# ilpoviertola/V-AURA

Measured on AMD Instinct MI355X. Metric: audio codec tokens/sec (whole node), 2.56 s clips, higher is better.
Workload: dtype f16x2-split(22b)/f32-acc

## Files before the change

include/vaura_hip.h:

```cpp
#ifndef VAURA_HIP_H
#define VAURA_HIP_H

#include <stddef.h>
#include <stdint.h>

#ifdef __cplusplus
extern "C" {
#endif

typedef void* vaura_stream_t;

typedef enum vaura_status {
  VAURA_OK = 0,
  VAURA_ERR_ARG = -1,
  VAURA_ERR_SHAPE = -2,
  VAURA_ERR_DTYPE = -3,
  VAURA_ERR_STATE = -4
} vaura_status;

typedef enum vaura_wdtype { VAURA_W_F32 = 0, VAURA_W_BF16 = 1, VAURA_W_FP8 = 2, VAURA_W_H1 = 3, VAURA_W_H2 = 4, VAURA_W_FP8H = 5 } vaura_wdtype;

typedef struct vaura_dims {
  int32_t n_layer;
  int32_t d_model;
// ... 213 lines not shown
  const vaura_vit_block* blocks_host;
  const float *norm_w, *norm_b;
  const float* agg_cls;
  const float *agg_ln1_w, *agg_ln1_b, *agg_ln2_w, *agg_ln2_b;
  const void* agg_in_w; const float* agg_in_b;
  const void* agg_out_w; const float* agg_out_b;
  const void* agg_l1_w; const float* agg_l1_b;
  const void* agg_l2_w; const float* agg_l2_b;
  float* ws_x; float* ws_qkv; uint16_t* ws_a; uint16_t* ws_h; uint16_t* ws_p; float* ws_z; float* ws_s;
} vaura_vit;
int vaura_avclip_forward(const vaura_vit* v, const float* frames, int n_seg, float* feats, vaura_stream_t s);
size_t vaura_avclip_workspace_bytes(const vaura_vit* v, int n_seg, int which);

void vaura_set_debug_flags(unsigned flags);
void vaura_set_debug_flags2(unsigned flags);
long long vaura_debug_counter(int which);

const char* vaura_version(void);
size_t vaura_struct_size(int which);

#ifdef __cplusplus
}
#endif
#endif
```

vaura_amd/_lib.py:

```python
from __future__ import annotations

import ctypes as C
import os
from typing import Optional

_HERE = os.path.dirname(os.path.abspath(__file__))
LIB_PATH = os.path.join(_HERE, "csrc", "libvaura_hip.so")

W_F32, W_BF16, W_FP8, W_H1, W_H2, W_FP8H = 0, 1, 2, 3, 4, 5
EPI_STORE, EPI_RESID, EPI_SWIGLU, EPI_GELU, EPI_LOGITS = 0, 1, 2, 3, 4
KERNEL_KINDS = ("embed", "qkv", "attn", "wo", "w13", "w2", "heads", "sample")

c_float_p = C.c_void_p


class Dims(C.Structure):
    _fields_ = [("n_layer", C.c_int32), ("d_model", C.c_int32), ("n_head", C.c_int32), ("ffn_dim", C.c_int32),
                ("n_codebooks", C.c_int32), ("vocab", C.c_int32), ("cond_dim", C.c_int32), ("tok_dim", C.c_int32),
                ("cond_in", C.c_int32), ("codebook_dim", C.c_int32), ("tokens_per_frame", C.c_int32),
                ("eps", C.c_float)]


class LayerWeights(C.Structure):
    _fields_ = [("wqkv", C.c_void_p), ("wo", C.c_void_p), ("w13", C.c_void_p), ("w2", C.c_void_p),
# ... 78 lines not shown

SIGNATURES = {
    "vaura_audio_normalize": (C.c_int, [C.c_void_p, C.c_void_p, C.c_int, C.c_int64, C.c_int, C.c_int, C.c_float, C.c_float,
                                        C.c_void_p, C.c_void_p]),
    "vaura_audio_scratch_elems": (C.c_size_t, [C.c_int]),
    "vaura_audio_loudness": (C.c_int, [C.c_void_p, C.c_void_p, C.c_int, C.c_int64, C.c_int, C.c_float, C.c_int, C.c_float, C.c_void_p,
                                       C.c_void_p]),
    "vaura_audio_loudness_scratch_elems": (C.c_size_t, [C.c_int]),
    "vaura_dac_encode": (C.c_int, [C.POINTER(CodecEncoder), C.c_void_p, C.c_int, C.c_int64, C.c_void_p, C.c_void_p]),
    "vaura_dac_encode_workspace_elems": (C.c_size_t, [C.POINTER(CodecEncoder), C.c_int, C.c_int64]),
    "vaura_avclip_forward": (C.c_int, [C.POINTER(Vit), C.c_void_p, C.c_int, C.c_void_p, C.c_void_p]),
    "vaura_avclip_workspace_bytes": (C.c_size_t, [C.POINTER(Vit), C.c_int, C.c_int]),
    "vaura_version": (C.c_char_p, []),
    "vaura_set_debug_flags": (None, [C.c_uint]),
    "vaura_set_debug_flags2": (None, [C.c_uint]),
    "vaura_debug_counter": (C.c_longlong, [C.c_int]),
    "vaura_struct_size": (C.c_size_t, [C.c_int]),
    "vaura_packed_weight_bytes": (C.c_size_t, [C.c_int64, C.c_int64, C.c_int]),
    "vaura_pack_weight": (C.c_int, [C.c_void_p, C.c_void_p, C.c_int64, C.c_int64, C.c_int, C.c_void_p]),
    "vaura_build_token_table": (C.c_int, [C.c_void_p, C.c_void_p, C.c_void_p, C.c_void_p, C.c_int, C.c_int, C.c_int,
                                          C.c_int, C.c_void_p]),
    "vaura_pack_rows": (C.c_int, [C.c_void_p, C.c_void_p, C.c_int64, C.c_int64, C.c_void_p]),
    "vaura_unpack_rows": (C.c_int, [C.c_void_p, C.c_void_p, C.c_int64, C.c_int64, C.c_void_p]),
    "vaura_prefill_cond": (C.c_int, [C.POINTER(Dims), C.c_void_p, C.c_void_p, C.c_void_p, C.c_int, C.c_void_p,
                                     C.c_void_p, C.c_int64, C.c_void_p]),
    "vaura_pattern_build": (C.c_int, [C.c_void_p, C.c_void_p, C.c_int, C.c_int, C.c_int, C.c_int, C.c_void_p]),
    "vaura_pattern_revert": (C.c_int, [C.c_void_p, C.c_void_p, C.c_int, C.c_int, C.c_int, C.c_int, C.c_int, C.c_void_p]),
    "vaura_sample": (C.c_int, [C.c_void_p, C.c_int, C.c_int, C.c_int, C.POINTER(Sampling), C.c_void_p, C.c_int64,
                               C.c_void_p, C.c_void_p]),
    "vaura_decode_step": (C.c_int, [C.POINTER(Decoder), C.POINTER(Sampling), C.c_int, C.c_void_p]),
# ... 67 lines not shown
```

vaura_amd/csrc/api.hip:

```cpp
#include "common.h"
#include <algorithm>
#include "gemv3_kernel.h"
#include <vector>

enum { EPI_STORE = 0, EPI_RESID = 1, EPI_SWIGLU = 2, EPI_GELU = 3, EPI_LOGITS = 4 };

static int check_decoder(const vaura_decoder* d) {
  if (!d || !d->layers_host || !d->heads || !d->final_norm || !d->tok_emb || !d->tok_proj_w || !d->tok_proj_b ||
      !d->tok_table || !d->empty_video || !d->rope || !d->cond_proj || !d->kcache || !d->vcache || !d->seq || !d->state || !d->ws_h ||
      !d->ws_qkv || !d->ws_attn || !d->ws_ffn || !d->ws_logits)
    return VAURA_ERR_ARG;
  const vaura_dims& m = d->dims;
  if (m.d_model != 1536 || m.ffn_dim != 4096 || m.n_head != 16 || m.vocab != 1024) return VAURA_ERR_SHAPE;
  if (m.cond_dim + m.tok_dim != m.d_model) return VAURA_ERR_SHAPE;
  if (d->rows != d->batch && d->rows != 2 * d->batch) return VAURA_ERR_ARG;
  if (d->seq_len > d->max_len || d->batch <= 0) return VAURA_ERR_ARG;
  if (d->plane_shift < 0 || d->plane_shift > 24 || (d->plane_shift && !d->ws_h_split)) return VAURA_ERR_ARG;
  if (d->kv_dtype < 0 || d->kv_dtype > 2) return VAURA_ERR_ARG;
  if (d->kv_dtype != 0 && (d->max_len > 256 || !d->ws_h_split)) return VAURA_ERR_SHAPE;
  return 0;
}

thread_local int va_prof_kind = -1;
struct StepProfiler {
// ... 71 lines not shown
  const size_t kv_layer = (size_t)rows * H * (size_t)d->max_len * hd;
  float* qkv2 = (d->ws_qkv2 && (rows + 15) / 16 < 16) ? d->ws_qkv2 : nullptr;
  const bool mlp_engine = !(va_debug_flags_get() & 4u) && va_mlp_engine_eligible(d);
  const bool fuse_qkv = mlp_engine && qkv2 && !(va_debug_flags_get() & 0x2u);
  bool qkv_done = false;
#ifdef VAURA_EXPERIMENT_ENGINES
  const bool attn_wo = mlp_engine && rows <= 16 && H == 16 && d->max_len <= 256 && (va_debug_flags_get() & 0x1000u) && !(va_debug_flags_get() & 8u) &&
                       d->plane_shift == 0;
  const bool fuse_attn = fuse_qkv && rows <= 16 && H == 16 && hd == 96 && d->max_len <= 256 && d->ws_attn_split && !attn_wo && d->plane_shift == 0 &&
                         !(va_debug_flags_get() & 8u) && (va_debug_flags2_get() & 4u);
  const bool tail_engine = mlp_engine && rows <= 16 && (va_debug_flags_get() & 8u);
#else
  constexpr bool attn_wo = false, fuse_attn = false;
#endif
  bool attn_done = false;
  for (int l = 0; l < m.n_layer; ++l) {
    const vaura_layer_weights& L = d->layers_host[l];
    const float* next_attn_gain = (l + 1 < m.n_layer) ? d->layers_host[l + 1].attn_norm : d->final_norm;
    if (!qkv_done) {
      PROF_B(VAURA_K_QKV);
      Gemv3Args aq = g3(L.wqkv, d->ws_h_split, d->ws_ss, nullptr, d->ws_qkv, nullptr, nullptr, nullptr, d, 3 * D);
      aq.out2 = qkv2;
      rc = va_launch_gemv3(aq, 3 * D, D, E3_STORE, true, s);
      PROF_A(VAURA_K_QKV);
      if (rc) return rc;
    }
    qkv_done = false;
#ifdef VAURA_EXPERIMENT_ENGINES
    const Gemv3Args awo0 = g3(L.wo, d->ws_attn_split, nullptr, d->ws_h, d->ws_h, d->ws_h_split, L.ffn_norm, d->ws_ss, d, D);
#endif
// ... 27 lines not shown
      if (rc) return rc;
      continue;
    }
#endif
    if (!attn_wo) {
      PROF_B(VAURA_K_WO);
      rc = va_launch_gemv3(awo, D, D, E3_RESID, false, s);
      PROF_A(VAURA_K_WO);
      if (rc) return rc;
    }
    const Gemv3Args a13 = g3(L.w13, d->ws_h_split, d->ws_ss, nullptr, nullptr, d->ws_ffn_split, nullptr, nullptr, d, F);
    const Gemv3Args a2 = g3(L.w2, d->ws_ffn_split, nullptr, d->ws_h, d->ws_h, d->ws_h_split, next_attn_gain, d->ws_ss, d, D);
    if (mlp_engine) {
      Gemv3Args aqn;
      const bool with_qkv = fuse_qkv && l + 1 < m.n_layer;
      if (with_qkv) {
        aqn = g3(d->layers_host[l + 1].wqkv, d->ws_h_split, d->ws_ss, nullptr, d->ws_qkv, nullptr, nullptr, nullptr, d, 3 * D);
        aqn.out2 = qkv2;
      }
      VaEngineAttention att;
      const bool with_attn = with_qkv && fuse_attn;
      if (with_attn)
        att = VaEngineAttention{d->rope, d->kcache + (size_t)(l + 1) * kv_layer, d->vcache + (size_t)(l + 1) * kv_layer, d->ws_attn,
                                d->ws_attn_split, H, d->max_len};
      PROF_B(VAURA_K_W13);
      const void* warm = l + 1 < m.n_layer ? d->layers_host[l + 1].w13 : nullptr;
      const size_t warm_bytes = (size_t)2 * F * D * (d->wdtype == VAURA_W_H2 ? 4 : (va_is_fp8(d->wdtype) ? 1 : 2));
      rc = va_launch_mlp_engine(a13, a2, with_qkv ? &aqn : nullptr, d->ws_sync, d->state, l, s, with_attn ? &att : nullptr, warm, warm_bytes,
                                l + 1 < m.n_layer ? d->layers_host[l + 1].wo : nullptr, warm_bytes * D / (2 * F));
      PROF_A(VAURA_K_W13);
      if (rc) return rc;
      qkv_done = with_qkv;
      attn_done = with_attn;
      continue;
    }
    PROF_B(VAURA_K_W13);
    rc = va_launch_gemv3(a13, 2 * F, D, E3_SWIGLU, true, s);
    PROF_A(VAURA_K_W13);
    if (rc) return rc;
    PROF_B(VAURA_K_W2);
    rc = va_launch_gemv3(a2, D, F, E3_RESID, false, s);
    PROF_A(VAURA_K_W2);
    if (rc) return rc;
  }
  if (!sample) return va_launch_advance(d->state, -1, s);
  PROF_B(VAURA_K_HEADS);
  rc = va_launch_gemv3(g3(d->heads, d->ws_h_split, d->ws_ss, nullptr, d->ws_logits, nullptr, nullptr, nullptr, d,
                          m.n_codebooks * m.vocab), (int64_t)m.n_codebooks * m.vocab, D, E3_LOGITS, true, s);
  PROF_A(VAURA_K_HEADS);
  if (rc) return rc;
  PROF_B(VAURA_K_SAMPLE);
  rc = va_launch_sample(d->ws_logits, d->batch, m.n_codebooks, m.vocab, sp, d->noise, d->batch * m.n_codebooks, d->state, 0,
                        nullptr, d->seq, d->timesteps, d->seq_len, d->state, s);
  PROF_A(VAURA_K_SAMPLE);
  return rc;
}

static int enqueue_step(const vaura_decoder* d, const vaura_sampling* sp, int sample, hipStream_t s) {
  if (d->wdtype == VAURA_W_H1 || d->wdtype == VAURA_W_H2 || va_is_fp8(d->wdtype)) return enqueue_step_bf16(d, sp, sample, s);
  if (d->wdtype != VAURA_W_F32 && d->wdtype != VAURA_W_BF16) return VAURA_ERR_DTYPE;
  const vaura_dims& m = d->dims;
  const int D = m.d_model, F = m.ffn_dim, H = m.n_head, hd = D / H;
  const int rows = d->rows;
  PROF_B(VAURA_K_EMBED);
  int rc = va_launch_embed(d, -1, 1, s);
// ... 217 lines not shown
```

vaura_amd/csrc/common.h:

```cpp
#pragma once
#include <hip/hip_runtime.h>
#include <hip/hip_ext.h>
#include <stdint.h>
#include "../../include/vaura_hip.h"

typedef float f32x4 __attribute__((ext_vector_type(4)));
typedef uint32_t u32x4 __attribute__((ext_vector_type(4)));

#define VA_CHECK_LAUNCH()                      \
  do {                                         \
    hipError_t e__ = hipGetLastError();        \
    if (e__ != hipSuccess) return (int)e__;    \
  } while (0)
extern thread_local int va_prof_kind;
void va_prof_events(hipEvent_t* start, hipEvent_t* stop);
#define VA_LAUNCH(kern, grid, block, smem, stream, ...)                                              \
  do {                                                                                               \
    (void)hipGetLastError();                                                                         \
    if (va_prof_kind >= 0) {                                                                         \
      hipEvent_t va_e0, va_e1;                                                                       \
      va_prof_events(&va_e0, &va_e1);                                                                \
      hipExtLaunchKernelGGL(kern, grid, block, smem, stream, va_e0, va_e1, 0, __VA_ARGS__);         \
    } else {                                                                                         \
      hipLaunchKernelGGL(kern, grid, block, smem, stream, __VA_ARGS__);                              \
// ... 132 lines not shown
unsigned va_debug_flags_get();
int va_pack_weight_fp8(const float* src, void* dst, int64_t N, int64_t K, hipStream_t s);
int va_pack_weight_h(const float* src, void* dst, int64_t N, int64_t K, int planes, hipStream_t s);
int va_launch_gemv3(const Gemv3Args& a, int64_t n_weight_rows, int64_t K, int epilogue, bool norm, hipStream_t s);
bool va_mlp_engine_eligible(const vaura_decoder* d);
struct VaEngineAttention {
  const float* rope;
  float* kc;
  float* vc;
  float* out;
  uint16_t* outp;
  int n_head, max_len;
};
int va_launch_mlp_engine(const Gemv3Args& a13, const Gemv3Args& a2, const Gemv3Args* aq_next, uint32_t* flags, int32_t* state, int layer,
                         hipStream_t s, const VaEngineAttention* att = nullptr, const void* warm_ptr = nullptr, size_t warm_bytes = 0,
                         const void* warm0_ptr = nullptr, size_t warm0_bytes = 0);
int va_launch_attn_wo(const float* qkv, const float* qkv2, const float* rope, float* kc, float* vc, float* out, uint16_t* outp,
                      int rows, int n_head, int max_len, const int32_t* state, const Gemv3Args& awo, uint32_t* flags, int layer, hipStream_t s);
int va_launch_tail_engine(const Gemv3Args& awo, const Gemv3Args& a13, const Gemv3Args& a2, uint32_t* flags, int32_t* state, int layer,
                          hipStream_t s);
int va_launch_embed(const vaura_decoder* d, int pos_host, int n_pos, hipStream_t s);
int va_launch_sample(const float* logits, int B, int K, int vocab, const vaura_sampling* sp, const float* noise,
                     int noise_rows_per_step, const int32_t* state, int64_t step_host, int32_t* tokens_out,
                     int32_t* seq, int T, int S, int32_t* state_rw, hipStream_t s);
int va_launch_advance(int32_t* state, int set_to, hipStream_t s);
int va_launch_linear_pair(const uint16_t* in, const uint16_t* w, const float* bias, const float* res, float* out_raw,
                          uint16_t* out_act, int act, int B, int Lin, int Lout, int oshift, int Cin, int Cout, hipStream_t s);
int va_launch_rope_append(const vaura_decoder* d, int layer, int p0, int n_pos, hipStream_t s);
int va_launch_attention_prefill(const vaura_decoder* d, int layer, int p0, int n_pos, hipStream_t s);

__device__ __forceinline__ uint32_t va_handoff_epoch(const int32_t* state, int layer) {
// ... 3 lines not shown
```

vaura_amd/csrc/gemv3.hip:

```cpp
#include "gemv3_kernel.h"
#include "mlp_engine.h"
#include <cstdlib>

unsigned va_debug_flags = 0;
VA_STAMP_SETTER(vaura_stamps_set_gemv3)
unsigned va_debug_flags_get() { return va_debug_flags; }

unsigned va_debug_flags2 = 0;
unsigned va_debug_flags2_get() { return va_debug_flags2; }
static bool rb2(const Gemv3Args& a) { return a.R >= 2 && !(va_debug_flags2 & 1u); }

template <int WT, int G, int NW, int T, int EPI, bool NORM, int XB = 1, int KS = 1, bool RB2 = false, int XBR = XB>
static int launch3(const Gemv3Args& a, int64_t n_tiles, hipStream_t s) {
  if (n_tiles % T) return VAURA_ERR_SHAPE;
  if constexpr (RB2) {
    if (rb2(a)) {
      VA_LAUNCH((gemv3_kernel<G, NW, T, EPI, NORM, XBR, 0, WT, KS, 2>), dim3((unsigned)(n_tiles / T * KS)), dim3(NW * 64), 0, s, a.W, a.XP, a);
      return 0;
    }
  }
  VA_LAUNCH((gemv3_kernel<G, NW, T, EPI, NORM, XB, 0, WT, KS>), dim3((unsigned)(n_tiles / T * KS)), dim3(NW * 64), 0, s, a.W, a.XP, a);
  return 0;
}

// ... 166 lines not shown
  if (d->rows > 16 && (va_debug_flags2 & 2u)) return false;
  if (va_is_fp8(d->wdtype)) { if (d->rows <= 16 || (va_debug_flags2 & 16u)) return false; }
  else if (d->wdtype != VAURA_W_H1 && d->wdtype != VAURA_W_H2) return false;
  if (d->dims.d_model != 1536 || d->dims.ffn_dim != 4096) return false;
  static int cus[64] = {};
  int dev = 0;
  if (hipGetDevice(&dev) != hipSuccess || dev < 0 || dev >= 64) return false;
  if (!cus[dev]) {
    int n = 0;
    if (hipDeviceGetAttribute(&n, hipDeviceAttributeMultiprocessorCount, dev) != hipSuccess) return false;
    cus[dev] = n > 0 ? n : -1;
  }
  return cus[dev] >= 256;
}

template <int WT, bool QKV, int RBK = 1, bool ATT = false>
static int launch_mlp_engine_t(const MlpEngineArgs& e, hipStream_t s) {
  using SH = MlpEngineShape<WT, RBK>;
  static unsigned long long big = 0;
  if (va_big_lds_once(reinterpret_cast<const void*>(mlp_engine_kernel<WT, QKV, RBK, ATT>), SH::LDS, &big)) return VAURA_ERR_STATE;
  VA_LAUNCH((mlp_engine_kernel<WT, QKV, RBK, ATT>), dim3(256), dim3(MLPE_NW * 64), SH::LDS, s, e.p1.W, e.p1.XP, e.p2.W, e);
  return 0;
}

int va_launch_mlp_engine(const Gemv3Args& a13, const Gemv3Args& a2, const Gemv3Args* aq, uint32_t* flags, int32_t* state, int layer,
                         hipStream_t s, const VaEngineAttention* att, const void* warm_ptr, size_t warm_bytes, const void* warm0_ptr,
                         size_t warm0_bytes) {
  MlpEngineArgs e;
  const unsigned six = (va_debug_flags2 >> 16) & 31u;
  e.pf_ptr = static_cast<const unsigned char*>(warm_ptr);
  e.pf_lines = (warm_ptr && six) ? (int)((warm_bytes / 128) * (six > 16 ? 16 : six) / 16) : 0;
  e.pf_early = (int)((va_debug_flags2 >> 21) & 1u);
  e.pf_ptr0 = static_cast<const unsigned char*>(warm0_ptr);
  e.pf_lines0 = (warm0_ptr && (va_debug_flags2 & 0x400000u)) ? (int)(warm0_bytes / 128) : 0;
  e.att_rope = nullptr; e.att_kc = e.att_vc = e.att_out = nullptr; e.att_outp = nullptr; e.att_max_len = 0;
  if (att) {
    if (!aq || a13.R != 1 || !att->rope || !att->kc || !att->vc || !att->out || att->n_head != 16 || att->max_len > 256 || att->max_len < 1)
      return VAURA_ERR_ARG;
    e.att_rope = att->rope; e.att_kc = att->kc; e.att_vc = att->vc; e.att_out = att->out; e.att_outp = att->outp; e.att_max_len = att->max_len;
  }
  e.p1 = a13;
  e.p2 = a2;
  e.p3 = aq ? *aq : a2;
  if (aq) {
    if (!aq->W || !aq->out || !aq->out2 || !aq->ss_in || aq->XP != a2.outp || aq->ss_in != a2.ss_out || aq->R != a2.R) return VAURA_ERR_ARG;
    if (aq->wq != a2.wq || aq->N != 3 * 1536 || aq->k_total != 1536 || aq->n_ss_in != 96) return VAURA_ERR_SHAPE;
    e.p3.wscale = weight_scales(*aq, 3 * 1536, 1536);
  }
  if (!a13.W || !a13.XP || !a2.W || !a2.XP || !flags || !state || a13.R < 1 || a13.R > 2 || a2.R != a13.R) return VAURA_ERR_ARG;
  if (a13.wq != a2.wq || a13.wq < 0 || a13.wq > 3 || ((a13.wq == 1 || a13.wq == 3) && (a13.R != 2 || att)) || a13.N != 4096 || a2.N != 1536 || a13.k_total != 1536 ||
      a13.n_ss_in != 96) return VAURA_ERR_SHAPE;
  e.p1.wscale = weight_scales(a13, 2 * 4096, 1536);
  e.p2.wscale = weight_scales(a2, 1536, 4096);
  e.flags = flags; e.state = state; e.state_rw = state; e.layer = layer;
  e.abl = (int)((va_debug_flags >> 28) & 15u);
  e.qlocal = (int)((va_debug_flags2 >> 23) & 1u);
  e.pollwave = ((va_debug_flags2 >> 7) & 1u) && !(e.abl & 4);
  if (a13.R == 2) {
    if (a13.wq == 1) return aq ? launch_mlp_engine_t<1, true, 2>(e, s) : launch_mlp_engine_t<1, false, 2>(e, s);
    if (a13.wq == 3) return aq ? launch_mlp_engine_t<3, true, 2>(e, s) : launch_mlp_engine_t<3, false, 2>(e, s);
    if (aq) return a13.wq == 2 ? launch_mlp_engine_t<2, true, 2>(e, s) : launch_mlp_engine_t<0, true, 2>(e, s);
    return a13.wq == 2 ? launch_mlp_engine_t<2, false, 2>(e, s) : launch_mlp_engine_t<0, false, 2>(e, s);
  }
#ifdef VAURA_EXPERIMENT_ENGINES
  if (att) return a13.wq == 2 ? launch_mlp_engine_t<2, true, 1, true>(e, s) : launch_mlp_engine_t<0, true, 1, true>(e, s);
#else
  if (att) return VAURA_ERR_STATE;
#endif
  if (aq) return a13.wq == 2 ? launch_mlp_engine_t<2, true>(e, s) : launch_mlp_engine_t<0, true>(e, s);
  return a13.wq == 2 ? launch_mlp_engine_t<2, false>(e, s) : launch_mlp_engine_t<0, false>(e, s);
}

#ifdef VAURA_EXPERIMENT_ENGINES
template <int WT>
static int launch_tail_engine_t(const TailEngineArgs& e, hipStream_t s) {
  using SH = MlpEngineShape<WT>;
  static unsigned long long big = 0;
  if (va_big_lds_once(reinterpret_cast<const void*>(tail_engine_kernel<WT>), SH::LDS, &big)) return VAURA_ERR_STATE;
  VA_LAUNCH((tail_engine_kernel<WT>), dim3(256), dim3(MLPE_NW * 64), SH::LDS, s, e.p0.W, e.p0.XP, e.p1.W, e.p2.W, e);
  return 0;
}

int va_launch_tail_engine(const Gemv3Args& awo, const Gemv3Args& a13, const Gemv3Args& a2, uint32_t* flags, int32_t* state, int layer,
// ... 128 lines not shown
  f32x4 v = reinterpret_cast<const f32x4*>(src)[packed_quad(row, cq, C)];
  if (ss) {
    float s = ((v[0] * v[0] + v[1] * v[1]) + v[2] * v[2]) + v[3] * v[3];
    s += __shfl_xor(s, 1, 64);
    s += __shfl_xor(s, 2, 64);
    if ((cq & 3) == 0) ss[((size_t)(row >> 4) * (C / 16) + (cq >> 2)) * 16 + (row & 15)] = s;
  }
  if (gain) v *= *reinterpret_cast<const f32x4*>(gain + cq * 4);
  store_split4(dst, row, cq * 4, C, v);
}

extern "C" {

void vaura_set_debug_flags(unsigned flags) { va_debug_flags = flags; }
void vaura_set_debug_flags2(unsigned flags) { va_debug_flags2 = flags; }

int vaura_split_rows(const float* src, uint16_t* dst, const float* gain, float* ss, int64_t rows, int64_t C, vaura_stream_t s) {
  if (!src || !dst || rows <= 0 || C <= 0 || (C % 16)) return VAURA_ERR_ARG;
  const int rows_p = (int)((rows + 15) / 16 * 16);
  const int64_t total = (int64_t)rows_p * (C / 4);
  VA_LAUNCH(split_rows_kernel, dim3((unsigned)((total + 255) / 256)), dim3(256), 0, as_stream(s), src, dst, gain, ss, rows_p, (int)C);
  return 0;
}

int vaura_gemv_pair(const void* w, int wdtype, const uint16_t* x_split, const float* ss_in, int n_ss_in, const float* residual, float* out,
                    float* out_khalf2, uint16_t* out_split, const float* gain_out, float* ss_out, int64_t rows, int64_t N, int64_t K, int epilogue,
                    float eps, vaura_stream_t s) {
  if (!w || !x_split || rows <= 0) return VAURA_ERR_ARG;
  if (wdtype != VAURA_W_H1 && !va_is_fp8(wdtype) && wdtype != VAURA_W_H2) return VAURA_ERR_DTYPE;
  Gemv3Args a;
// ... 10 lines not shown
```

vaura_amd/csrc/mlp_engine.h:

```cpp
#pragma once
#include "gemv3_kernel.h"

#ifndef MLPE_REL
#define MLPE_REL 0
#endif
template <typename F>
__device__ __forceinline__ void va_static_for9(F&& f) {
  f(std::integral_constant<int, 0>{}); f(std::integral_constant<int, 1>{}); f(std::integral_constant<int, 2>{});
  f(std::integral_constant<int, 3>{}); f(std::integral_constant<int, 4>{}); f(std::integral_constant<int, 5>{});
  f(std::integral_constant<int, 6>{}); f(std::integral_constant<int, 7>{}); f(std::integral_constant<int, 8>{});
}
template <int WT, int RBK = 1>
struct MlpeThrottle {
#ifdef MLPE_Q2
  static constexpr int Q2_1 = MLPE_Q2;
#else
  static constexpr int Q2_1 = WT == 2 ? 2 : 1;
#endif
#ifdef MLPE_PRE3
  static constexpr int PRE3 = MLPE_PRE3;
#else
  static constexpr int PRE3 = WT == 2 ? 1 : 2;
#endif
#ifdef MLPE_PRE3U
  static constexpr int PRE3U_1 = MLPE_PRE3U;
#else
// ... 11 lines not shown
#endif
  static constexpr int Q2 = RBK == 2 ? Q2_2 : Q2_1;
  static constexpr int PRE3U = RBK == 2 ? PRE3U_2 : PRE3U_1;
};
struct MlpEngineArgs {
  Gemv3Args p1;
  Gemv3Args p2;
  Gemv3Args p3;
  uint32_t* flags;
  const int32_t* state;
  int32_t* state_rw;
  int layer;
  int abl;
  int qlocal;
  int pollwave;
  const unsigned char* pf_ptr;
  int pf_lines;
  const unsigned char* pf_ptr0;
  int pf_lines0;
  int pf_early;
  const float* att_rope;
  float* att_kc;
  float* att_vc;
  float* att_out;
  uint16_t* att_outp;
  int att_max_len;
};

#define MLPE_NW 8
#define MLPE_SPIN_LIMIT 20000
// ... 42 lines not shown
      if (lane == 0) __hip_atomic_fetch_or(e.state_rw + 4, VAURA_STATUS_HANDOFF_TIMEOUT, __ATOMIC_RELAXED, __HIP_MEMORY_SCOPE_AGENT);
      broken = true;
      break;
    }
    __builtin_amdgcn_s_sleep(2);
  }
  return broken;
}

__device__ __forceinline__ uint32_t mlpe_ld_sc1(const uint32_t* p) {
  uint32_t v;
  asm volatile("global_load_dword %0, %1, off sc1\n\ts_waitcnt vmcnt(0)" : "=&v"(v) : "v"(p) : "memory");
  return v;
}

template <int WT, bool QKV, int RBK = 1, bool ATT = false>
__global__ __launch_bounds__(MLPE_NW * 64) void mlp_engine_kernel(const void* __restrict__ W13q, const uint16_t* __restrict__ XPq,
                                                                  const void* __restrict__ W2q, MlpEngineArgs e) {
  using SH = MlpEngineShape<WT, RBK>;
  constexpr bool F32 = WTag<WT>::F32, FP8 = WTag<WT>::FP8;
  constexpr int XPL = WTag<WT>::XPL;
  static_assert(!FP8 || (RBK == 2 && !ATT), "fp8 tile pairs: the two-row-block instances only (configs[4]'s shape)");
  constexpr int WH = SH::WH, NW = MLPE_NW, NACC = 2;
  extern __shared__ __attribute__((aligned(16))) unsigned char mlpe_lds[];
  unsigned char* ring = mlpe_lds;
  f32x4* red = reinterpret_cast<f32x4*>(mlpe_lds + NW * SH::WAVE_RING);
  unsigned* arrive = reinterpret_cast<unsigned*>(mlpe_lds + NW * SH::WAVE_RING + SH::RED);
  unsigned* arrive2 = arrive + NW;

  VA_STAMP_DECL(stamps);
  VA_STAMP(stamps, 0);
  const int lane = threadIdx.x & 63;
  const int wid = __builtin_amdgcn_readfirstlane(threadIdx.x >> 6);
  const int bid = blockIdx.x;
  const uint32_t epoch = va_handoff_epoch(e.state, e.layer);
  const uint32_t ltag = epoch ^ ((uint32_t)(blockIdx.x + 1) * 0x9E3779B1u);

// ... 571 lines not shown
      if (epw && wid * 16 < a.rows) {
        const int m = lane & 15;
        const bool mine = (m >> 3) == h;
        const int src = (m & 7) + 16 * (q & 1);
        f32x4 v = red[((wid * NW + 0) * 2 + (q >> 1)) * 64 + src];
#pragma unroll
        for (int i = 1; i < NW; ++i) v += red[((wid * NW + i) * 2 + (q >> 1)) * 64 + src];
        v *= ws2;
        if (mine) gemv3_epilogue<1, E3_RESID>(a, wid, tile, lane, &v, &pre);
      }
      VA_WAIT_VM(0);
      VA_STAMP(stamps, 6);
      VA_STAMP_FLUSH(stamps, 11);
    } else {
      Gemv3Args aq = e.p3;
      constexpr int G = FP8 ? 6 : 3, NWQ = FP8 ? 4 : NW, GF = 3, TQ = 3, KQ = 1536, KGQ = KQ / 32;
#ifdef MLPE_ATT_LOCAL
      const int qid = ATT ? (((bid >> 3) % 12) >> 2) * 64 + 4 * ((bid & 7) + 8 * ((bid >> 3) / 12)) + (((bid >> 3) % 12) & 3) : bid;
#elif defined(VAURA_EXPERIMENT_ENGINES)
      const int qid = (!ATT && e.qlocal) ? (((bid >> 3) % 12) >> 2) * 64 + 4 * ((bid & 7) + 8 * ((bid >> 3) / 12)) + (((bid >> 3) % 12) & 3) : bid;
#else
      const int qid = bid;
#endif
      const int ks = qid & 1, tile0q = (qid >> 1) * TQ, kgo = ks * G * NWQ;
      const bool actq = wid < NWQ;
      const int w3 = (wid + bid) % NWQ;
      const int mq = lane & 15;
      const int lane16 = lane * 16;
      const __amdgpu_buffer_rsrc_t qrs = __builtin_amdgcn_make_buffer_rsrc(const_cast<void*>(aq.W), 0, -16, 0x00020000);
      u32x4 wq[TQ][GF][WH];
      auto wq_off = [&](int t, int f, int hh) {
        const size_t kg = FP8 ? (size_t)(tile0q + t) * (KGQ / 2) + (size_t)((kgo + w3 * G + 2 * f) >> 1)
                              : ((size_t)(tile0q + t) * KGQ + (size_t)(kgo + w3 * G + f)) * WH + hh;
        return (int)(kg * 1024);
      };
      auto load_wq_g = [&](auto gc) {
        constexpr int g = decltype(gc)::value;
#pragma unroll
        for (int t = 0; t < TQ; ++t) {
#pragma unroll
          for (int hh = 0; hh < WH; ++hh)
            wq[t][g][hh] = __builtin_amdgcn_raw_buffer_load_b128(qrs, lane16, wq_off(t, g, hh), 2 );
        }
      };
      auto load_wq = [&]() {
        if (!actq) return;
        load_wq_g(std::integral_constant<int, 0>{});
        load_wq_g(std::integral_constant<int, 1>{});
        load_wq_g(std::integral_constant<int, 2>{});
      };
      if (lane == 0) __hip_atomic_store(arrive2 + wid, ltag, __ATOMIC_RELEASE, __HIP_MEMORY_SCOPE_WORKGROUP);
#ifdef MLPE_DIAG2
      VA_STAMP(stamps, 1);
#endif
      f32x4 wsq = f32x4{1.f, 1.f, 1.f, 1.f};
      const bool epq = wid < TQ * RBK;
      const int rq = wid / TQ, tq = wid - rq * TQ;
      if (!epw && actq) {
        if (!(e.abl & 8)) {
          constexpr int PRE3U = MlpeThrottle<WT, RBK>::PRE3U;
          auto unit = [&](auto uc) {
            constexpr int u = decltype(uc)::value, g = u / 3, t = u % 3;
#pragma unroll
            for (int hh = 0; hh < WH; ++hh)
              wq[t][g][hh] = __builtin_amdgcn_raw_buffer_load_b128(qrs, lane16, wq_off(t, g, hh), 2 );
          };
          va_static_for9([&](auto uc) { if constexpr (decltype(uc)::value < PRE3U) unit(uc); });
          if (PRE3U < 9)
            while (__hip_atomic_load(arrive + 17, __ATOMIC_ACQUIRE, __HIP_MEMORY_SCOPE_WORKGROUP) != ltag) __builtin_amdgcn_s_sleep(1);
          va_static_for9([&](auto uc) { if constexpr (decltype(uc)::value >= PRE3U) unit(uc); });
        } else {
          load_wq();
        }
      }
      if (epq) wsq = *reinterpret_cast<const f32x4*>(aq.wscale + (size_t)(tile0q + tq) * 16 + 4 * q);
      if (epw) {
        mlpe_wait_words(arrive2, ltag);
        const int m = lane & 15;
        const bool mine = (m >> 3) == h;
        const int src = (m & 7) + 16 * (q & 1);
        f32x4 v = red[((wid * NW + 0) * 2 + (q >> 1)) * 64 + src];
#pragma unroll
        for (int i = 1; i < NW; ++i) v += red[((wid * NW + i) * 2 + (q >> 1)) * 64 + src];
        v *= ws2;
        if (mine && wid * 16 < a.rows) gemv3_epilogue<1, E3_RESID>(a, wid, tile, lane, &v, &pre);
// ... 46 lines not shown
#pragma unroll
      for (int r = 0; r < RBK; ++r)
#pragma unroll
        for (int t = 0; t < TQ; ++t)
#pragma unroll
          for (int p = 0; p < NACC; ++p) accq[r][t][p] = f32x4{0.f, 0.f, 0.f, 0.f};
      if (actq) {
#pragma unroll
      for (int g = 0; g < G; ++g) {
#pragma unroll
        for (int t = 0; t < TQ; ++t) {
          f16x8 wf[F32 ? 2 : 1];
          if constexpr (FP8) {
            const u32x4 pr = wq[t][g / 2][0];
            wf[0] = (g & 1) ? fp8x8_to_f16(pr.z, pr.w) : fp8x8_to_f16(pr.x, pr.y);
          } else {
            wf[0] = __builtin_bit_cast(f16x8, wq[t][g][0]);
            if constexpr (F32) wf[1] = __builtin_bit_cast(f16x8, wq[t][g][WH - 1]);
          }
#pragma unroll
          for (int r = 0; r < RBK; ++r) mfma_group<WT>(wf, xq[r][g], accq[r][t]);
        }
        __builtin_amdgcn_sched_barrier(0);
      }
      }
      if (actq) {
#pragma unroll
        for (int r = 0; r < RBK; ++r)
#pragma unroll
          for (int t = 0; t < TQ; ++t) red[((r * NW + wid) * TQ + t) * 64 + lane] = acc_sum<WT>(accq[r][t]);
      }
      float rinvq = 1.f;
      if (epq) {
// ... 7 lines not shown
      if (ATT && !epq) att_request();
      __syncthreads();
      if (epq && rq * 16 < aq.rows) {
        f32x4 sacc = red[((rq * NW + 0) * TQ + tq) * 64 + lane];
#pragma unroll
        for (int i = 1; i < NWQ; ++i) sacc += red[((rq * NW + i) * TQ + tq) * 64 + lane];
        sacc *= wsq;
        const f32x4 v = sacc * rinvq;
        if (ks > 0) aq.out = aq.out2;
#ifdef MLPE_ATT_LOCAL
        if constexpr (ATT) {
          reinterpret_cast<f32x4*>(aq.out)[((size_t)rq * (aq.N / 4) + (size_t)(tile0q + tq) * 4) * 16 + lane] = v;
        } else
#endif
#ifdef VAURA_EXPERIMENT_ENGINES
        if (!ATT && e.qlocal) {
          reinterpret_cast<f32x4*>(aq.out)[((size_t)rq * (aq.N / 4) + (size_t)(tile0q + tq) * 4) * 16 + lane] = v;
        } else
#endif
        gemv3_epilogue<1, E3_STORE>(aq, rq, tile0q + tq, lane, &v, nullptr);
      }
      if constexpr (ATT) {
        if (epq) {
          asm volatile("s_waitcnt vmcnt(0)" ::: "memory");
          if (wid > 0) {
            if (lane == 0) __hip_atomic_store(arrive + 20 + wid, ltag, __ATOMIC_RELEASE, __HIP_MEMORY_SCOPE_WORKGROUP);
          } else {
            while (__hip_atomic_load(arrive + 21, __ATOMIC_ACQUIRE, __HIP_MEMORY_SCOPE_WORKGROUP) != ltag ||
                   __hip_atomic_load(arrive + 22, __ATOMIC_ACQUIRE, __HIP_MEMORY_SCOPE_WORKGROUP) != ltag)
              __builtin_amdgcn_s_sleep(1);
#ifdef MLPE_ATT_LOCAL
            if (lane == 0) asm volatile("global_store_dword %0, %1, off" ::"v"(e.flags + 512 + qid), "v"(epoch) : "memory");
#else
            if (lane == 0) asm volatile("global_store_dword %0, %1, off sc0 sc1" ::"v"(e.flags + 512 + qid), "v"(epoch) : "memory");
#endif
// ... 18 lines not shown
```

Measured before the change: 74590.

## Fuse output heads GEMV into final-layer MLP engine kernel

On the last layer, the persistent MLP engine kernel now runs the logits heads GEMV as its trailing phase, in the slot normally used for the next layer's QKV projection. The separate heads launch is then skipped. To fit the larger K range per block, some weight fragments are staged into the LDS ring through global_load_lds instead of registers, and a tunable prefetch count is added. This removes one kernel launch and its ramp-up from every decode step, at the cost of more register and LDS pressure and extra synchronisation inside the engine kernel.

```diff
diff --git a/include/vaura_hip.h b/include/vaura_hip.h
--- a/include/vaura_hip.h
+++ b/include/vaura_hip.h
@@ -251,6 +251,7 @@
 
 void vaura_set_debug_flags(unsigned flags);
 void vaura_set_debug_flags2(unsigned flags);
+int vaura_mlp_engine_heads_eligible(int rows, int wdtype, int64_t n_logits);
 long long vaura_debug_counter(int which);
 
 const char* vaura_version(void);
diff --git a/vaura_amd/_lib.py b/vaura_amd/_lib.py
--- a/vaura_amd/_lib.py
+++ b/vaura_amd/_lib.py
@@ -116,6 +116,7 @@
     "vaura_version": (C.c_char_p, []),
     "vaura_set_debug_flags": (None, [C.c_uint]),
     "vaura_set_debug_flags2": (None, [C.c_uint]),
+    "vaura_mlp_engine_heads_eligible": (C.c_int, [C.c_int, C.c_int, C.c_int64]),
     "vaura_debug_counter": (C.c_longlong, [C.c_int]),
     "vaura_struct_size": (C.c_size_t, [C.c_int]),
     "vaura_packed_weight_bytes": (C.c_size_t, [C.c_int64, C.c_int64, C.c_int]),
diff --git a/vaura_amd/csrc/api.hip b/vaura_amd/csrc/api.hip
--- a/vaura_amd/csrc/api.hip
+++ b/vaura_amd/csrc/api.hip
@@ -109,6 +109,8 @@
   constexpr bool attn_wo = false, fuse_attn = false;
 #endif
   bool attn_done = false;
+  const bool fuse_heads = sample && mlp_engine && va_mlp_engine_heads_eligible(rows, d->wdtype, (int64_t)m.n_codebooks * m.vocab);
+  bool heads_done = false;
   for (int l = 0; l < m.n_layer; ++l) {
     const vaura_layer_weights& L = d->layers_host[l];
     const float* next_attn_gain = (l + 1 < m.n_layer) ? d->layers_host[l + 1].attn_norm : d->final_norm;
@@ -166,9 +168,12 @@
     if (mlp_engine) {
       Gemv3Args aqn;
       const bool with_qkv = fuse_qkv && l + 1 < m.n_layer;
+      const bool with_heads = fuse_heads && l + 1 == m.n_layer;
       if (with_qkv) {
         aqn = g3(d->layers_host[l + 1].wqkv, d->ws_h_split, d->ws_ss, nullptr, d->ws_qkv, nullptr, nullptr, nullptr, d, 3 * D);
         aqn.out2 = qkv2;
+      } else if (with_heads) {
+        aqn = g3(d->heads, d->ws_h_split, d->ws_ss, nullptr, d->ws_logits, nullptr, nullptr, nullptr, d, m.n_codebooks * m.vocab);
       }
       VaEngineAttention att;
       const bool with_attn = with_qkv && fuse_attn;
@@ -178,11 +183,12 @@
       PROF_B(VAURA_K_W13);
       const void* warm = l + 1 < m.n_layer ? d->layers_host[l + 1].w13 : nullptr;
       const size_t warm_bytes = (size_t)2 * F * D * (d->wdtype == VAURA_W_H2 ? 4 : (va_is_fp8(d->wdtype) ? 1 : 2));
-      rc = va_launch_mlp_engine(a13, a2, with_qkv ? &aqn : nullptr, d->ws_sync, d->state, l, s, with_attn ? &att : nullptr, warm, warm_bytes,
-                                l + 1 < m.n_layer ? d->layers_host[l + 1].wo : nullptr, warm_bytes * D / (2 * F));
+      rc = va_launch_mlp_engine(a13, a2, (with_qkv || with_heads) ? &aqn : nullptr, d->ws_sync, d->state, l, s, with_attn ? &att : nullptr, warm,
+                                warm_bytes, l + 1 < m.n_layer ? d->layers_host[l + 1].wo : nullptr, warm_bytes * D / (2 * F), with_heads);
       PROF_A(VAURA_K_W13);
       if (rc) return rc;
       qkv_done = with_qkv;
+      heads_done = with_heads;
       attn_done = with_attn;
       continue;
     }
@@ -196,11 +202,13 @@
     if (rc) return rc;
   }
   if (!sample) return va_launch_advance(d->state, -1, s);
-  PROF_B(VAURA_K_HEADS);
-  rc = va_launch_gemv3(g3(d->heads, d->ws_h_split, d->ws_ss, nullptr, d->ws_logits, nullptr, nullptr, nullptr, d,
-                          m.n_codebooks * m.vocab), (int64_t)m.n_codebooks * m.vocab, D, E3_LOGITS, true, s);
-  PROF_A(VAURA_K_HEADS);
-  if (rc) return rc;
+  if (!heads_done) {
+    PROF_B(VAURA_K_HEADS);
+    rc = va_launch_gemv3(g3(d->heads, d->ws_h_split, d->ws_ss, nullptr, d->ws_logits, nullptr, nullptr, nullptr, d,
+                            m.n_codebooks * m.vocab), (int64_t)m.n_codebooks * m.vocab, D, E3_LOGITS, true, s);
+    PROF_A(VAURA_K_HEADS);
+    if (rc) return rc;
+  }
   PROF_B(VAURA_K_SAMPLE);
   rc = va_launch_sample(d->ws_logits, d->batch, m.n_codebooks, m.vocab, sp, d->noise, d->batch * m.n_codebooks, d->state, 0,
                         nullptr, d->seq, d->timesteps, d->seq_len, d->state, s);
diff --git a/vaura_amd/csrc/common.h b/vaura_amd/csrc/common.h
--- a/vaura_amd/csrc/common.h
+++ b/vaura_amd/csrc/common.h
@@ -170,7 +170,8 @@
 };
 int va_launch_mlp_engine(const Gemv3Args& a13, const Gemv3Args& a2, const Gemv3Args* aq_next, uint32_t* flags, int32_t* state, int layer,
                          hipStream_t s, const VaEngineAttention* att = nullptr, const void* warm_ptr = nullptr, size_t warm_bytes = 0,
-                         const void* warm0_ptr = nullptr, size_t warm0_bytes = 0);
+                         const void* warm0_ptr = nullptr, size_t warm0_bytes = 0, bool heads = false);
+bool va_mlp_engine_heads_eligible(int rows, int wdtype, int64_t n_logits);
 int va_launch_attn_wo(const float* qkv, const float* qkv2, const float* rope, float* kc, float* vc, float* out, uint16_t* outp,
                       int rows, int n_head, int max_len, const int32_t* state, const Gemv3Args& awo, uint32_t* flags, int layer, hipStream_t s);
 int va_launch_tail_engine(const Gemv3Args& awo, const Gemv3Args& a13, const Gemv3Args& a2, uint32_t* flags, int32_t* state, int layer,
diff --git a/vaura_amd/csrc/gemv3.hip b/vaura_amd/csrc/gemv3.hip
--- a/vaura_amd/csrc/gemv3.hip
+++ b/vaura_amd/csrc/gemv3.hip
@@ -1,5 +1,6 @@
 #include "gemv3_kernel.h"
 #include "mlp_engine.h"
+#include <algorithm>
 #include <cstdlib>
 
 unsigned va_debug_flags = 0;
@@ -204,19 +205,30 @@
   return cus[dev] >= 256;
 }
 
-template <int WT, bool QKV, int RBK = 1, bool ATT = false>
+template <int WT, bool QKV, int RBK = 1, bool ATT = false, bool HEADS = false>
 static int launch_mlp_engine_t(const MlpEngineArgs& e, hipStream_t s) {
   using SH = MlpEngineShape<WT, RBK>;
   static unsigned long long big = 0;
-  if (va_big_lds_once(reinterpret_cast<const void*>(mlp_engine_kernel<WT, QKV, RBK, ATT>), SH::LDS, &big)) return VAURA_ERR_STATE;
-  VA_LAUNCH((mlp_engine_kernel<WT, QKV, RBK, ATT>), dim3(256), dim3(MLPE_NW * 64), SH::LDS, s, e.p1.W, e.p1.XP, e.p2.W, e);
-  return 0;
+  if (va_big_lds_once(reinterpret_cast<const void*>(mlp_engine_kernel<WT, QKV, RBK, ATT, HEADS>), SH::LDS, &big)) return VAURA_ERR_STATE;
+  VA_LAUNCH((mlp_engine_kernel<WT, QKV, RBK, ATT, HEADS>), dim3(256), dim3(MLPE_NW * 64), SH::LDS, s, e.p1.W, e.p1.XP, e.p2.W, e);
+  return 0;
+}
+
+bool va_mlp_engine_heads_eligible(int rows, int wdtype, int64_t n_logits) {
+  return rows >= 1 && rows <= 16 && (wdtype == VAURA_W_H1 || wdtype == VAURA_W_H2) && n_logits == 192 * 3 * 16 && !(va_debug_flags2 & 256u);
 }
 
 int va_launch_mlp_engine(const Gemv3Args& a13, const Gemv3Args& a2, const Gemv3Args* aq, uint32_t* flags, int32_t* state, int layer,
                          hipStream_t s, const VaEngineAttention* att, const void* warm_ptr, size_t warm_bytes, const void* warm0_ptr,
-                         size_t warm0_bytes) {
+                         size_t warm0_bytes, bool heads) {
   MlpEngineArgs e;
+  const unsigned hv = (va_debug_flags2 >> 25) & 31u;
+  e.hpre = hv ? (int)std::min(hv - 1u, 18u) : (a13.wq == 2 ? 9 : 6);
+  if (heads) {
+    if (!aq || att || a13.R != 1 || (a13.wq != 0 && a13.wq != 2)) return VAURA_ERR_ARG;
+    if (!aq->W || !aq->out || !aq->ss_in || aq->XP != a2.outp || aq->ss_in != a2.ss_out || aq->R != 1) return VAURA_ERR_ARG;
+    if (aq->wq != a2.wq || aq->N != 192 * 3 * 16 || aq->k_total != 1536 || aq->n_ss_in != 96 || aq->out2) return VAURA_ERR_SHAPE;
+  }
   const unsigned six = (va_debug_flags2 >> 16) & 31u;
   e.pf_ptr = static_cast<const unsigned char*>(warm_ptr);
   e.pf_lines = (warm_ptr && six) ? (int)((warm_bytes / 128) * (six > 16 ? 16 : six) / 16) : 0;
@@ -232,7 +244,9 @@
   e.p1 = a13;
   e.p2 = a2;
   e.p3 = aq ? *aq : a2;
-  if (aq) {
+  if (aq && heads) {
+    e.p3.wscale = weight_scales(*aq, aq->N, 1536);
+  } else if (aq) {
     if (!aq->W || !aq->out || !aq->out2 || !aq->ss_in || aq->XP != a2.outp || aq->ss_in != a2.ss_out || aq->R != a2.R) return VAURA_ERR_ARG;
     if (aq->wq != a2.wq || aq->N != 3 * 1536 || aq->k_total != 1536 || aq->n_ss_in != 96) return VAURA_ERR_SHAPE;
     e.p3.wscale = weight_scales(*aq, 3 * 1536, 1536);
@@ -257,6 +271,7 @@
 #else
   if (att) return VAURA_ERR_STATE;
 #endif
+  if (heads) return a13.wq == 2 ? launch_mlp_engine_t<2, true, 1, false, true>(e, s) : launch_mlp_engine_t<0, true, 1, false, true>(e, s);
   if (aq) return a13.wq == 2 ? launch_mlp_engine_t<2, true>(e, s) : launch_mlp_engine_t<0, true>(e, s);
   return a13.wq == 2 ? launch_mlp_engine_t<2, false>(e, s) : launch_mlp_engine_t<0, false>(e, s);
 }
@@ -415,6 +430,7 @@
 
 void vaura_set_debug_flags(unsigned flags) { va_debug_flags = flags; }
 void vaura_set_debug_flags2(unsigned flags) { va_debug_flags2 = flags; }
+int vaura_mlp_engine_heads_eligible(int rows, int wdtype, int64_t n_logits) { return va_mlp_engine_heads_eligible(rows, wdtype, n_logits) ? 1 : 0; }
 
 int vaura_split_rows(const float* src, uint16_t* dst, const float* gain, float* ss, int64_t rows, int64_t C, vaura_stream_t s) {
   if (!src || !dst || rows <= 0 || C <= 0 || (C % 16)) return VAURA_ERR_ARG;
diff --git a/vaura_amd/csrc/mlp_engine.h b/vaura_amd/csrc/mlp_engine.h
--- a/vaura_amd/csrc/mlp_engine.h
+++ b/vaura_amd/csrc/mlp_engine.h
@@ -1,4 +1,5 @@
 #pragma once
+#include <utility>
 #include "gemv3_kernel.h"
 
 #ifndef MLPE_REL
@@ -10,6 +11,10 @@
   f(std::integral_constant<int, 3>{}); f(std::integral_constant<int, 4>{}); f(std::integral_constant<int, 5>{});
   f(std::integral_constant<int, 6>{}); f(std::integral_constant<int, 7>{}); f(std::integral_constant<int, 8>{});
 }
+template <typename F, int... I>
+__device__ __forceinline__ void va_static_for_impl(F& f, std::integer_sequence<int, I...>) { (f(std::integral_constant<int, I>{}), ...); }
+template <int N, typename F>
+__device__ __forceinline__ void va_static_for(F&& f) { va_static_for_impl(f, std::make_integer_sequence<int, N>{}); }
 template <int WT, int RBK = 1>
 struct MlpeThrottle {
 #ifdef MLPE_Q2
@@ -51,6 +56,7 @@
   int abl;
   int qlocal;
   int pollwave;
+  int hpre;
   const unsigned char* pf_ptr;
   int pf_lines;
   const unsigned char* pf_ptr0;
@@ -123,13 +129,14 @@
   return v;
 }
 
-template <int WT, bool QKV, int RBK = 1, bool ATT = false>
+template <int WT, bool QKV, int RBK = 1, bool ATT = false, bool HEADS = false>
 __global__ __launch_bounds__(MLPE_NW * 64) void mlp_engine_kernel(const void* __restrict__ W13q, const uint16_t* __restrict__ XPq,
                                                                   const void* __restrict__ W2q, MlpEngineArgs e) {
   using SH = MlpEngineShape<WT, RBK>;
   constexpr bool F32 = WTag<WT>::F32, FP8 = WTag<WT>::FP8;
   constexpr int XPL = WTag<WT>::XPL;
   static_assert(!FP8 || (RBK == 2 && !ATT), "fp8 tile pairs: the two-row-block instances only (configs[4]'s shape)");
+  static_assert(!HEADS || (QKV && RBK == 1 && !ATT && !FP8), "the heads phase: one row block, fp16-plane weights (the heads are never fp8)");
   constexpr int WH = SH::WH, NW = MLPE_NW, NACC = 2;
   extern __shared__ __attribute__((aligned(16))) unsigned char mlpe_lds[];
   unsigned char* ring = mlpe_lds;
@@ -731,41 +738,47 @@
       VA_STAMP_FLUSH(stamps, 11);
     } else {
       Gemv3Args aq = e.p3;
-      constexpr int G = FP8 ? 6 : 3, NWQ = FP8 ? 4 : NW, GF = 3, TQ = 3, KQ = 1536, KGQ = KQ / 32;
+      constexpr int G = (FP8 || HEADS) ? 6 : 3, NWQ = FP8 ? 4 : NW, GF = HEADS ? 6 : 3, TQ = 3, KQ = 1536, KGQ = KQ / 32;
+      constexpr int HRING = (HEADS && WT == 2) ? 2 : 0, GR = GF - HRING;
+      static_assert(HRING * TQ * WH <= SH::NF, "the ring holds the heads fragments that do not travel in registers");
+      unsigned char* myring = ring + wid * SH::WAVE_RING;
 #ifdef MLPE_ATT_LOCAL
       const int qid = ATT ? (((bid >> 3) % 12) >> 2) * 64 + 4 * ((bid & 7) + 8 * ((bid >> 3) / 12)) + (((bid >> 3) % 12) & 3) : bid;
 #elif defined(VAURA_EXPERIMENT_ENGINES)
-      const int qid = (!ATT && e.qlocal) ? (((bid >> 3) % 12) >> 2) * 64 + 4 * ((bid & 7) + 8 * ((bid >> 3) / 12)) + (((bid >> 3) % 12) & 3) : bid;
+      const int qid = (!ATT && !HEADS && e.qlocal) ? (((bid >> 3) % 12) >> 2) * 64 + 4 * ((bid & 7) + 8 * ((bid >> 3) / 12)) + (((bid >> 3) % 12) & 3) : bid;
 #else
       const int qid = bid;
 #endif
-      const int ks = qid & 1, tile0q = (qid >> 1) * TQ, kgo = ks * G * NWQ;
+      const int ks = HEADS ? 0 : (qid & 1), tile0q = (HEADS ? qid : (qid >> 1)) * TQ, kgo = ks * G * NWQ;
       const bool actq = wid < NWQ;
       const int w3 = (wid + bid) % NWQ;
       const int mq = lane & 15;
       const int lane16 = lane * 16;
       const __amdgpu_buffer_rsrc_t qrs = __builtin_amdgcn_make_buffer_rsrc(const_cast<void*>(aq.W), 0, -16, 0x00020000);
-      u32x4 wq[TQ][GF][WH];
+      u32x4 wq[TQ][GR][WH];
       auto wq_off = [&](int t, int f, int hh) {
         const size_t kg = FP8 ? (size_t)(tile0q + t) * (KGQ / 2) + (size_t)((kgo + w3 * G + 2 * f) >> 1)
                               : ((size_t)(tile0q + t) * KGQ + (size_t)(kgo + w3 * G + f)) * WH + hh;
         return (int)(kg * 1024);
       };
-      auto load_wq_g = [&](auto gc) {
-        constexpr int g = decltype(gc)::value;
-#pragma unroll
-        for (int t = 0; t < TQ; ++t) {
-#pragma unroll
-          for (int hh = 0; hh < WH; ++hh)
+      auto wq_unit = [&](auto uc) {
+        constexpr int u = decltype(uc)::value, g = u / TQ, t = u % TQ;
+#pragma unroll
+        for (int hh = 0; hh < WH; ++hh) {
+          if constexpr (g < GR) {
             wq[t][g][hh] = __builtin_amdgcn_raw_buffer_load_b128(qrs, lane16, wq_off(t, g, hh), 2 );
+          } else {
+            const unsigned char* src = static_cast<const unsigned char*>(aq.W) + wq_off(t, g, hh) + lane16;
+            __builtin_amdgcn_global_load_lds((const __attribute__((address_space(1))) void*)src,
+                                             (__attribute__((address_space(3))) void*)(myring + (((g - GR) * TQ + t) * WH + hh) * 1024), 16, 0, 2 );
+          }
         }
       };
       auto load_wq = [&]() {
         if (!actq) return;
-        load_wq_g(std::integral_constant<int, 0>{});
-        load_wq_g(std::integral_constant<int, 1>{});
-        load_wq_g(std::integral_constant<int, 2>{});
+        va_static_for<GF * TQ>(wq_unit);
       };
+      if constexpr (HRING > 0) asm volatile("s_waitcnt lgkmcnt(0)" ::: "memory");
       if (lane == 0) __hip_atomic_store(arrive2 + wid, ltag, __ATOMIC_RELEASE, __HIP_MEMORY_SCOPE_WORKGROUP);
 #ifdef MLPE_DIAG2
       VA_STAMP(stamps, 1);
@@ -775,17 +788,19 @@
       const int rq = wid / TQ, tq = wid - rq * TQ;
       if (!epw && actq) {
         if (!(e.abl & 8)) {
-          constexpr int PRE3U = MlpeThrottle<WT, RBK>::PRE3U;
-          auto unit = [&](auto uc) {
-            constexpr int u = decltype(uc)::value, g = u / 3, t = u % 3;
-#pragma unroll
-            for (int hh = 0; hh < WH; ++hh)
-              wq[t][g][hh] = __builtin_amdgcn_raw_buffer_load_b128(qrs, lane16, wq_off(t, g, hh), 2 );
-          };
-          va_static_for9([&](auto uc) { if constexpr (decltype(uc)::value < PRE3U) unit(uc); });
-          if (PRE3U < 9)
-            while (__hip_atomic_load(arrive + 17, __ATOMIC_ACQUIRE, __HIP_MEMORY_SCOPE_WORKGROUP) != ltag) __builtin_amdgcn_s_sleep(1);
-          va_static_for9([&](auto uc) { if constexpr (decltype(uc)::value >= PRE3U) unit(uc); });
+          if constexpr (HEADS) {
+            const int npre = e.hpre;
+            va_static_for<GF * TQ>([&](auto uc) { if (decltype(uc)::value < npre) wq_unit(uc); });
+            if (npre < GF * TQ)
+              while (__hip_atomic_load(arrive + 17, __ATOMIC_ACQUIRE, __HIP_MEMORY_SCOPE_WORKGROUP) != ltag) __builtin_amdgcn_s_sleep(1);
+            va_static_for<GF * TQ>([&](auto uc) { if (decltype(uc)::value >= npre) wq_unit(uc); });
+          } else {
+            constexpr int PRE3U = MlpeThrottle<WT, RBK>::PRE3U;
+            va_static_for9([&](auto uc) { if constexpr (decltype(uc)::value < PRE3U) wq_unit(uc); });
+            if (PRE3U < 9)
+              while (__hip_atomic_load(arrive + 17, __ATOMIC_ACQUIRE, __HIP_MEMORY_SCOPE_WORKGROUP) != ltag) __builtin_amdgcn_s_sleep(1);
+            va_static_for9([&](auto uc) { if constexpr (decltype(uc)::value >= PRE3U) wq_unit(uc); });
+          }
         } else {
           load_wq();
         }
@@ -862,9 +877,14 @@
           if constexpr (FP8) {
             const u32x4 pr = wq[t][g / 2][0];
             wf[0] = (g & 1) ? fp8x8_to_f16(pr.z, pr.w) : fp8x8_to_f16(pr.x, pr.y);
+          } else if (g < GR) {
+            wf[0] = __builtin_bit_cast(f16x8, wq[t][g < GR ? g : 0][0]);
+            if constexpr (F32) wf[1] = __builtin_bit_cast(f16x8, wq[t][g < GR ? g : 0][WH - 1]);
           } else {
-            wf[0] = __builtin_bit_cast(f16x8, wq[t][g][0]);
-            if constexpr (F32) wf[1] = __builtin_bit_cast(f16x8, wq[t][g][WH - 1]);
+            if (t == 0 && g == GR) asm volatile("s_waitcnt vmcnt(0)" ::: "memory");
+            const unsigned char* fr = myring + ((g - GR) * TQ + t) * WH * 1024 + lane16;
+            wf[0] = __builtin_bit_cast(f16x8, *reinterpret_cast<const u32x4*>(fr));
+            if constexpr (F32) wf[1] = __builtin_bit_cast(f16x8, *reinterpret_cast<const u32x4*>(fr + (WH - 1) * 1024));
           }
 #pragma unroll
           for (int r = 0; r < RBK; ++r) mfma_group<WT>(wf, xq[r][g], accq[r][t]);
@@ -902,11 +922,12 @@
         } else
 #endif
 #ifdef VAURA_EXPERIMENT_ENGINES
-        if (!ATT && e.qlocal) {
+        if (!ATT && !HEADS && e.qlocal) {
           reinterpret_cast<f32x4*>(aq.out)[((size_t)rq * (aq.N / 4) + (size_t)(tile0q + tq) * 4) * 16 + lane] = v;
         } else
 #endif
-        gemv3_epilogue<1, E3_STORE>(aq, rq, tile0q + tq, lane, &v, nullptr);
+        if constexpr (HEADS) gemv3_epilogue<1, E3_LOGITS>(aq, rq, tile0q + tq, lane, &v, nullptr);
+        else gemv3_epilogue<1, E3_STORE>(aq, rq, tile0q + tq, lane, &v, nullptr);
       }
       if constexpr (ATT) {
         if (epq) {
```

Result: no change. 74800, median of 6 (+0.3%).
